# dgaddy/silent_speech

Measured on AMD Instinct MI355X. Metric: EMG frames/s training (transduction_model.py), higher is better.
Workload: dtype bf16

## Files before the change

### silent_speech_amd/csrc/loss.hip

```cpp
#include "common.h"
#include <stdlib.h>
#include "silent_speech_hip.h"
#include <math.h>

namespace {
constexpr int DESC = 10;
enum { D_N = 0, D_M, D_PRED_ROW0, D_TGT_ROW0, D_UNUSED, D_SK_OFF, D_DIRS_OFF, D_BND_OFF, D_RES_OFF };
constexpr int DW = 4, DR = 4;
__device__ __forceinline__ long long dtw_strips_d(long long n) { long long rows = n - 1, cap = DW * 64 * DR; return rows <= 0 ? 0 : (rows + cap - 1) / cap; }
__device__ __forceinline__ long long dtw_tsteps_d(long long m) { return m <= 1 ? 0 : (m - 1) + 63; }
}

__global__ void frame_lse_kernel(const float* __restrict__ head, long long ld, int col0, int ncls, int rows, float* __restrict__ lse, int* __restrict__ amax)
{
    const int lane = threadIdx.x & 63, wpb = blockDim.x >> 6;
    for (int r = blockIdx.x * wpb + (threadIdx.x >> 6); r < rows; r += gridDim.x * wpb) {
        const float* a = head + (long long)r * ld + col0;
        float mx = -INFINITY; int mi = 0x7fffffff;
        for (int c = lane; c < ncls; c += 64) { float v = a[c]; if (v > mx) { mx = v; mi = c; } }
        const float gmx = wave_max(mx);
        int cand = (mx == gmx) ? mi : 0x7fffffff;
#pragma unroll
        for (int m = 32; m >= 1; m >>= 1) { int o = __shfl_xor(cand, m); cand = o < cand ? o : cand; }
        float s = 0.f;
        for (int c = lane; c < ncls; c += 64) s += expf(a[c] - gmx);
        s = wave_sum(s);
        if (lane == 0) { lse[r] = gmx + logf(s); amax[r] = cand; }
    }
}

extern "C" int ss_frame_lse(const float* head, int64_t ld, int col0, int ncls, int rows, float* lse, int32_t* argmax, void* stream)
{
    SS_CHECK(head && lse && argmax, "ss_frame_lse: null pointer");
    if (rows <= 0) return 0;
    int blocks = (rows + 3) / 4; if (blocks > 4096) blocks = 4096;
    SS_LAUNCH(frame_lse_kernel, dim3(blocks), dim3(256), 0, stream, head, (long long)ld, col0, ncls, rows, lse, argmax);
    SS_LAUNCH_CHECK("ss_frame_lse");
    return 0;
}

constexpr int UTT = 8;
__global__ void loss_index_tables_kernel(const long long* __restrict__ utt, int* __restrict__ vo_pred, int* __restrict__ vo_tgt,
                                         int* __restrict__ si_tgt, int* __restrict__ si_base, int* __restrict__ si_res)
{
    const long long* u = utt + (long long)blockIdx.x * UTT;
    const int n1 = (int)u[0], n2 = (int)u[1];
    const int p0 = (int)u[3], t0 = (int)u[4], r0 = (int)u[5];
    if (u[2]) {
        const long long o = u[7];
        for (int i = threadIdx.x; i < n2; i += blockDim.x) { si_tgt[o + i] = t0 + i; si_base[o + i] = p0; si_res[o + i] = r0 + i; }
    } else {
        const long long o = u[6];
        for (int i = threadIdx.x; i < n1; i += blockDim.x) { vo_pred[o + i] = p0 + i; vo_tgt[o + i] = t0 + i; }
    }
}

extern "C" int ss_loss_index_tables(const int64_t* utt_dev, int n_utt, int32_t* vo_pred, int32_t* vo_tgt, int32_t* si_tgt, int32_t* si_base,
                                    int32_t* si_res, void* stream)
{
    SS_CHECK(n_utt >= 0, "ss_loss_index_tables: negative utterance count");
    if (n_utt == 0) return 0;
    SS_CHECK(utt_dev && vo_pred && vo_tgt && si_tgt && si_base && si_res, "ss_loss_index_tables: null pointer");
    SS_LAUNCH(loss_index_tables_kernel, dim3((unsigned)n_utt), dim3(256), 0, stream, (const long long*)utt_dev, (int*)vo_pred, (int*)vo_tgt, (int*)si_tgt,
              (int*)si_base, (int*)si_res);
    SS_LAUNCH_CHECK("ss_loss_index_tables");
    return 0;
}

__device__ __forceinline__ void loss_block_commit(float lsum, int csum, float inv_total, float* loss_acc, int* correct_acc)
{
    __shared__ float ls[16];
    __shared__ int cs[16];
    const int lane = threadIdx.x & 63, w = threadIdx.x >> 6, wpb = blockDim.x >> 6;
    if (lane == 0) { ls[w] = lsum; cs[w] = csum; }
    __syncthreads();
    if (threadIdx.x == 0) {
        float a = 0.f; int c = 0;
        for (int i = 0; i < wpb; ++i) { a += ls[i]; c += cs[i]; }
        if (a != 0.f) atomicAdd(loss_acc, a * inv_total);
        if (c) atomicAdd(correct_acc, c);
    }
}

__global__ void voiced_loss_kernel(const float* __restrict__ head, long long ld, int n_mel, int n_ph, const float* __restrict__ lse, const int* __restrict__ amax,
                                   const float* __restrict__ Y, const long long* __restrict__ phones, const int* __restrict__ pred_row, const int* __restrict__ tgt_row,
                                   int nframes, float lam, float inv_total, float* __restrict__ dhead, float* __restrict__ loss_acc, int* __restrict__ correct_acc)
{
    const int lane = threadIdx.x & 63, wpb = blockDim.x >> 6;
    float lsum = 0.f; int csum = 0;
    for (int f = blockIdx.x * wpb + (threadIdx.x >> 6); f < nframes; f += gridDim.x * wpb) {
        const int pr = pred_row[f], tr = tgt_row[f];
        const float* p = head + (long long)pr * ld; const float* y = Y + (long long)tr * n_mel;
        float* dp = dhead + (long long)pr * ld;
        float ss = 0.f;
        for (int c = lane; c < n_mel; c += 64) { float d = y[c] - p[c] + 1e-6f; ss += d * d; }
        const float dist = sqrtf(wave_sum(ss));
        const float gs = dist > 0.f ? inv_total / dist : 0.f;
        for (int c = lane; c < n_mel; c += 64) dp[c] = -(y[c] - p[c] + 1e-6f) * gs;
        const int ph = (int)phones[tr];
        const float L = lse[pr];
        for (int c = lane; c < n_ph; c += 64) dp[n_mel + c] = lam * inv_total * (expf(p[n_mel + c] - L) - (c == ph ? 1.f : 0.f));
        if (lane == 0) { lsum += dist + lam * (L - p[n_mel + ph]); csum += amax[pr] == ph; }
    }
    loss_block_commit(lsum, csum, inv_total, loss_acc, correct_acc);
}

extern "C" int ss_voiced_loss(const float* head, int64_t ld, int n_mel, int n_phone, const float* lse, const int32_t* argmax, const float* Y, const int64_t* phones,
                              const int32_t* pred_row, const int32_t* tgt_row, int nframes, float lam, float inv_total,
                              float* dhead, float* loss_accum, int32_t* correct_accum, void* stream)
{
    SS_CHECK(nframes >= 0, "ss_voiced_loss: negative frame count");
    if (nframes == 0) return 0;
    SS_CHECK(head && lse && argmax && Y && phones && pred_row && tgt_row && dhead && loss_accum && correct_accum, "ss_voiced_loss: null pointer");
    int blocks = (nframes + 3) / 4; if (blocks > 1024) blocks = 1024;
    SS_LAUNCH(voiced_loss_kernel, dim3(blocks), dim3(256), 0, stream, head, (long long)ld, n_mel, n_phone, lse, (const int*)argmax, Y, (const long long*)phones,
              (const int*)pred_row, (const int*)tgt_row, nframes, lam, inv_total, dhead, loss_accum, (int*)correct_accum);
    SS_LAUNCH_CHECK("ss_voiced_loss");
    return 0;
}

constexpr int YMAX = 128;
__device__ __forceinline__ float quad_bcast(float v, int k) {
#if defined(SS_EMU)
    return __shfl(v, (int)((threadIdx.x & 63) & ~3) + k);
#else
    switch (k) {
    case 0: return __int_as_float(__builtin_amdgcn_update_dpp(0, __float_as_int(v), 0x00, 0xf, 0xf, true));
    case 1: return __int_as_float(__builtin_amdgcn_update_dpp(0, __float_as_int(v), 0x55, 0xf, 0xf, true));
    case 2: return __int_as_float(__builtin_amdgcn_update_dpp(0, __float_as_int(v), 0xAA, 0xf, 0xf, true));
    default: return __int_as_float(__builtin_amdgcn_update_dpp(0, __float_as_int(v), 0xFF, 0xf, 0xf, true));
    }
#endif
}
template <int NQ>
__device__ __forceinline__ float quad_shared_sqdist(const float* __restrict__ p, int r, const f32x4 (&yv)[YMAX / 4]) {
    f32x4 own[NQ];
#pragma unroll
    for (int q = 0; q < NQ; ++q) own[q] = *(const f32x4*)(p + (r * NQ + q) * 4);
    float ss = 0.f;
#pragma unroll
    for (int k = 0; k < 4; ++k) {
#pragma unroll
        for (int q = 0; q < NQ; ++q) {
            const f32x4 b = yv[k * NQ + q];
            const float a0 = quad_bcast(own[q][0], k), a1 = quad_bcast(own[q][1], k), a2 = quad_bcast(own[q][2], k), a3 = quad_bcast(own[q][3], k);
            const float d0 = a0 - b[0], d1 = a1 - b[1], d2 = a2 - b[2], d3 = a3 - b[3];
            ss += d0 * d0; ss += d1 * d1; ss += d2 * d2; ss += d3 * d3;
        }
    }
    return ss;
}

__global__ __launch_bounds__(256) void silent_cost_skewed_kernel(const float* __restrict__ head, long long ld, int n_mel, const float* __restrict__ lse, const float* __restrict__ Y,
                                                                 const long long* __restrict__ phones, const long long* __restrict__ desc, float lam, unsigned char* __restrict__ ws, int* __restrict__ results, int CT)
{
    const long long* d = desc + (long long)blockIdx.y * DESC;
    const int N = (int)d[D_N], M = (int)d[D_M];
    const long long p0 = d[D_PRED_ROW0], y0 = d[D_TGT_ROW0];
    int* res = results + d[D_RES_OFF];
    for (int i = blockIdx.x * blockDim.x + threadIdx.x; i < N; i += gridDim.x * blockDim.x) res[i] = 0;
    const long long ts = dtw_tsteps_d(M), nkw = dtw_strips_d(N) * DW;
    if (ts <= 0) return;
    const long long tchunks = (ts + CT - 1) / CT, nwork = nkw * tchunks;
    float* sk = (float*)(ws + d[D_SK_OFF]);
    const int l = threadIdx.x >> 2, r = threadIdx.x & 3;
    for (long long wk = blockIdx.x; wk < nwork; wk += gridDim.x) {
        const long long kw = wk / tchunks, t0 = (wk - kw * tchunks) * CT;
        const long long i = 1 + (kw * 64 + l) * DR + r;
        const bool iv = i < N;
        f32x4 yv[YMAX / 4];
        int ph = 0;
        if (iv) {
            const float* y = Y + (y0 + i) * n_mel;
#pragma unroll
            for (int q = 0; q < YMAX / 4; ++q) if (q * 4 < n_mel) yv[q] = *(const f32x4*)(y + q * 4);
            ph = (int)phones[y0 + i];
        }
        const long long tend = t0 + CT < ts ? t0 + CT : ts;
        if (n_mel == 80) {
            for (long long t = t0; t < tend; ++t) {
                const long long j = t + 1 - l;
                const bool jv = j >= 1 && j < M;
                const float* p = head + (p0 + (jv ? j : 1)) * ld;
                const float ss = quad_shared_sqdist<5>(p, r, yv);
                float c = INFINITY;
                if (jv && iv) c = sqrtf(ss) + lam * (lse[p0 + j] - p[n_mel + ph]);
                sk[((kw * ts + t) * 64 + l) * DR + r] = c;
            }
            continue;
        }
        for (long long t = t0; t < tend; ++t) {
            const long long j = t + 1 - l;
            float c = INFINITY;
            if (iv && j >= 1 && j < M) {
                const float* p = head + (p0 + j) * ld;
                float ss = 0.f;
#pragma unroll
                for (int q = 0; q < YMAX / 4; ++q) {
                    if (q * 4 < n_mel) {
                        const f32x4 a = *(const f32x4*)(p + q * 4), b = yv[q];
                        const float d0 = a[0] - b[0], d1 = a[1] - b[1], d2 = a[2] - b[2], d3 = a[3] - b[3];
                        ss += d0 * d0; ss += d1 * d1; ss += d2 * d2; ss += d3 * d3;
                    }
                }
                c = sqrtf(ss) + lam * (lse[p0 + j] - p[n_mel + ph]);
            }
            sk[((kw * ts + t) * 64 + l) * DR + r] = c;
        }
    }
}

extern "C" int ss_silent_cost_skewed(const float* head, int64_t ld, int n_mel, const float* lse, const float* Y, const int64_t* phones,
                                     const int64_t* desc_dev, int n, int max_n, int max_m, float lam, void* workspace, int32_t* results, void* stream)
{
    SS_CHECK(n >= 0, "ss_silent_cost_skewed: negative batch");
    if (n == 0) return 0;
    SS_CHECK(head && lse && Y && phones && desc_dev && workspace && results, "ss_silent_cost_skewed: null pointer");
    SS_CHECK(n_mel % 4 == 0 && ld % 4 == 0, "ss_silent_cost_skewed: n_mel and ld must be multiples of 4 (16-byte rows)");
    SS_CHECK(n_mel <= YMAX, "ss_silent_cost_skewed: at most %d mel bins", YMAX);
    long long strips = max_n <= 1 ? 0 : (max_n - 1 + DW * 64 * DR - 1) / (DW * 64 * DR);
    const long long ts_max = max_m <= 1 ? 0 : max_m - 1 + 63;
    static const int CT = getenv("SS_COST_CT") ? atoi(getenv("SS_COST_CT")) : 16;
    long long blocks = strips * DW * ((ts_max + CT - 1) / CT);
    if (blocks < (max_n + 255) / 256) blocks = (max_n + 255) / 256;
    if (blocks > 4096) blocks = 4096;
    if (blocks < 1) blocks = 1;
    SS_LAUNCH(silent_cost_skewed_kernel, dim3((unsigned)blocks, n), dim3(256), 0, stream, head, (long long)ld, n_mel, lse, Y, (const long long*)phones,
              (const long long*)desc_dev, lam, (unsigned char*)workspace, (int*)results, CT);
    SS_LAUNCH_CHECK("ss_silent_cost_skewed");
    return 0;
}

__global__ void silent_loss_kernel(const float* __restrict__ head, long long ld, int n_mel, int n_ph, const float* __restrict__ lse, const int* __restrict__ amax,
                                   const float* __restrict__ Y, const long long* __restrict__ phones, const int* __restrict__ results,
                                   const int* __restrict__ tgt_row, const int* __restrict__ pred_base, const int* __restrict__ res_idx,
                                   int nframes, float lam, float inv_total, float* __restrict__ dhead, float* __restrict__ loss_acc, int* __restrict__ correct_acc)
{
    const int lane = threadIdx.x & 63, wpb = blockDim.x >> 6;
    float lsum = 0.f; int csum = 0;
    for (int f = blockIdx.x * wpb + (threadIdx.x >> 6); f < nframes; f += gridDim.x * wpb) {
        const int tr = tgt_row[f], pr = pred_base[f] + results[res_idx[f]];
        const float* p = head + (long long)pr * ld; const float* y = Y + (long long)tr * n_mel;
        float* dp = dhead + (long long)pr * ld;
        float ss = 0.f;
        for (int c = lane; c < n_mel; c += 64) { float d = p[c] - y[c]; ss += d * d; }
        const float dist = sqrtf(wave_sum(ss));
        const float gs = dist > 0.f ? inv_total / dist : 0.f;
        for (int c = lane; c < n_mel; c += 64) atomicAdd(dp + c, (p[c] - y[c]) * gs);
        const int ph = (int)phones[tr];
        const float L = lse[pr];
        for (int c = lane; c < n_ph; c += 64) atomicAdd(dp + n_mel + c, lam * inv_total * (expf(p[n_mel + c] - L) - (c == ph ? 1.f : 0.f)));
        if (lane == 0) { lsum += dist + lam * (L - p[n_mel + ph]); csum += amax[pr] == ph; }
    }
    loss_block_commit(lsum, csum, inv_total, loss_acc, correct_acc);
}

extern "C" int ss_silent_loss(const float* head, int64_t ld, int n_mel, int n_phone, const float* lse, const int32_t* argmax, const float* Y, const int64_t* phones,
                              const int32_t* results, const int32_t* tgt_row, const int32_t* pred_base, const int32_t* res_idx, int nframes,
                              float lam, float inv_total, float* dhead, float* loss_accum, int32_t* correct_accum, void* stream)
{
    SS_CHECK(nframes >= 0, "ss_silent_loss: negative frame count");
    if (nframes == 0) return 0;
    SS_CHECK(head && lse && argmax && Y && phones && results && tgt_row && pred_base && res_idx && dhead && loss_accum && correct_accum, "ss_silent_loss: null pointer");
    int blocks = (nframes + 3) / 4; if (blocks > 1024) blocks = 1024;
    SS_LAUNCH(silent_loss_kernel, dim3(blocks), dim3(256), 0, stream, head, (long long)ld, n_mel, n_phone, lse, (const int*)argmax, Y, (const long long*)phones,
              (const int*)results, (const int*)tgt_row, (const int*)pred_base, (const int*)res_idx, nframes, lam, inv_total, dhead, loss_accum, (int*)correct_accum);
    SS_LAUNCH_CHECK("ss_silent_loss");
    return 0;
}

__global__ void phoneme_confusion_kernel(const int* __restrict__ amax, const long long* __restrict__ phones, const int* __restrict__ results,
                                         const int* __restrict__ vo_pred, const int* __restrict__ vo_tgt, int n_voiced,
                                         const int* __restrict__ si_tgt, const int* __restrict__ si_base, const int* __restrict__ si_res, int n_silent,
                                         int* __restrict__ conf, int n_phone)
{
    for (int i = blockIdx.x * blockDim.x + threadIdx.x; i < n_voiced + n_silent; i += gridDim.x * blockDim.x) {
        int p, t;
        if (i < n_voiced) { p = amax[vo_pred[i]]; t = (int)phones[vo_tgt[i]]; }
        else { const int k = i - n_voiced; p = amax[si_base[k] + results[si_res[k]]]; t = (int)phones[si_tgt[k]]; }
        if ((unsigned)p < (unsigned)n_phone && (unsigned)t < (unsigned)n_phone) atomicAdd(conf + p * n_phone + t, 1);
        else atomicAdd(conf + n_phone * n_phone, 1);
    }
}

extern "C" int ss_phoneme_confusion(const int32_t* argmax, const int64_t* phones, const int32_t* results, const int32_t* vo_pred, const int32_t* vo_tgt,
                                    int n_voiced, const int32_t* si_tgt, const int32_t* si_base, const int32_t* si_res, int n_silent_frames,
                                    int32_t* confusion, int n_phone, void* stream)
{
    SS_CHECK(argmax && phones && confusion, "ss_phoneme_confusion: null pointer");
    SS_CHECK(n_voiced == 0 || (vo_pred && vo_tgt), "ss_phoneme_confusion: voiced tables missing");
    SS_CHECK(n_silent_frames == 0 || (results && si_tgt && si_base && si_res), "ss_phoneme_confusion: silent tables missing");
    const int n = n_voiced + n_silent_frames;
    if (n <= 0) return 0;
    int blocks = (n + 255) / 256; if (blocks > 1024) blocks = 1024;
    SS_LAUNCH(phoneme_confusion_kernel, dim3(blocks), dim3(256), 0, stream, argmax, (const long long*)phones, results, vo_pred, vo_tgt, n_voiced,
              si_tgt, si_base, si_res, n_silent_frames, confusion, n_phone);
    SS_LAUNCH_CHECK("ss_phoneme_confusion");
    return 0;
}
```

### silent_speech_amd/csrc/runtime.hip

```cpp
#include "common.h"
#include "silent_speech_hip.h"
#include <stdarg.h>

static thread_local char g_err[512] = "";

void ss_set_error(const char* fmt, ...) {
    va_list ap; va_start(ap, fmt);
    vsnprintf(g_err, sizeof(g_err), fmt, ap);
    va_end(ap);
}
extern "C" const char* ss_last_error(void) { return g_err; }
extern "C" int ss_abi_version(void) { return SS_ABI_VERSION; }
extern "C" const char* ss_target_arch(void) {
#if defined(SS_EMU)
    return "host-emulator";
#else
    return "gfx950";
#endif
}
int ss_check_launch(const char* what) {
    hipError_t e = hipGetLastError();
    if (e != hipSuccess) { ss_set_error("%s: kernel launch failed: %s", what, hipGetErrorString(e)); return 2; }
    return 0;
}

#if !defined(SS_EMU)
#include <mutex>
namespace {
struct PinnedRing {
    static constexpr int N = 8;
    void* buf[N] = {}; size_t cap[N] = {}; hipEvent_t ev[N] = {}; bool used[N] = {}; int at = 0; std::mutex mu;
};
PinnedRing g_ring;
}
#endif
int ss_upload_table(void* dst_dev, const void* src_host, size_t bytes, void* stream)
{
    if (bytes == 0) return 0;
#if defined(SS_EMU)
    memcpy(dst_dev, src_host, bytes);
    return 0;
#else
    std::lock_guard<std::mutex> lock(g_ring.mu);
    const int i = g_ring.at; g_ring.at = (i + 1) % PinnedRing::N;
    if (g_ring.used[i] && hipEventSynchronize(g_ring.ev[i]) != hipSuccess) { ss_set_error("table upload: event wait failed"); return 1; }
    if (g_ring.cap[i] < bytes) {
        if (g_ring.buf[i]) (void)hipHostFree(g_ring.buf[i]);
        size_t cap = 1 << 16; while (cap < bytes) cap <<= 1;
        if (hipHostMalloc(&g_ring.buf[i], cap, hipHostMallocDefault) != hipSuccess) { g_ring.buf[i] = nullptr; g_ring.cap[i] = 0; ss_set_error("table upload: pinned allocation of %zu bytes failed", cap); return 1; }
        g_ring.cap[i] = cap;
    }
    if (!g_ring.ev[i] && hipEventCreateWithFlags(&g_ring.ev[i], hipEventDisableTiming) != hipSuccess) { ss_set_error("table upload: event creation failed"); return 1; }
    memcpy(g_ring.buf[i], src_host, bytes);
    if (hipMemcpyAsync(dst_dev, g_ring.buf[i], bytes, hipMemcpyHostToDevice, (hipStream_t)stream) != hipSuccess) { ss_set_error("table upload failed"); return 1; }
    if (hipEventRecord(g_ring.ev[i], (hipStream_t)stream) != hipSuccess) { ss_set_error("table upload: event record failed"); return 1; }
    g_ring.used[i] = true;
    return 0;
#endif
}

template <class TI, class TO>
__global__ void permute3d_kernel(const TI* __restrict__ in, TO* __restrict__ out, int d0, int d1, int d2,
                                 long long s0, long long s1, long long s2, int valid1, int valid2, float scale, int accumulate)
{
    long long total = (long long)d0 * d1 * d2;
    for (long long i = (long long)blockIdx.x * blockDim.x + threadIdx.x; i < total; i += (long long)gridDim.x * blockDim.x) {
        int c = (int)(i % d2); long long t = i / d2; int b = (int)(t % d1); int a = (int)(t / d1);
        float v = (b < valid1 && c < valid2) ? ldf(in + a * s0 + b * s1 + c * s2) * scale : 0.f;
        if (accumulate) v += ldf(out + i);
        stf(out + i, v);
    }
}

extern "C" int ss_permute3d(const void* in, int in_dtype, void* out, int out_dtype, int d0, int d1, int d2,
                            int64_t s0, int64_t s1, int64_t s2, int valid1, int valid2, float scale, int accumulate, void* stream)
{
    SS_CHECK(in && out, "ss_permute3d: null pointer");
    SS_CHECK(d0 >= 0 && d1 >= 0 && d2 >= 0, "ss_permute3d: negative extent");
    long long total = (long long)d0 * d1 * d2;
    if (total == 0) return 0;
    int block = 256; long long g = (total + block - 1) / block; if (g > 4096) g = 4096;
    dim3 grid((unsigned)g), blk(block);
#define SS_P3(TI, TO) SS_LAUNCH(SS_KERNEL(permute3d_kernel<TI, TO>), grid, blk, 0, stream, (const TI*)in, (TO*)out, d0, d1, d2, (long long)s0, (long long)s1, (long long)s2, valid1, valid2, scale, accumulate)
    if (in_dtype == SS_F32 && out_dtype == SS_F32) SS_P3(float, float);
    else if (in_dtype == SS_F32 && out_dtype == SS_BF16) SS_P3(float, bf16_t);
    else if (in_dtype == SS_BF16 && out_dtype == SS_F32) SS_P3(bf16_t, float);
    else if (in_dtype == SS_BF16 && out_dtype == SS_BF16) SS_P3(bf16_t, bf16_t);
    else SS_CHECK(false, "ss_permute3d: bad dtype");
#undef SS_P3
    SS_LAUNCH_CHECK("ss_permute3d");
    return 0;
}

struct PermuteJob {
    const void* in; void* out;
    long long s0, s1, s2, o0, o1;
    int d0, d1, d2, valid1, valid2, in_dtype, out_dtype, accumulate;
    float scale; int first_block, nblocks, pad_;
};

template <class TI> struct Vec4;
template <> struct Vec4<float> { static __device__ __forceinline__ void load(const float* p, float (&v)[4]) { const f32x4 a = *(const f32x4*)p; v[0] = a[0]; v[1] = a[1]; v[2] = a[2]; v[3] = a[3]; } };
template <> struct Vec4<bf16_t> { static __device__ __forceinline__ void load(const bf16_t* p, float (&v)[4]) { const u32x2 a = *(const u32x2*)p; v[0] = __uint_as_float(a[0] << 16); v[1] = __uint_as_float(a[0] & 0xffff0000u); v[2] = __uint_as_float(a[1] << 16); v[3] = __uint_as_float(a[1] & 0xffff0000u); } };

template <class TI, class TO, bool GROUPED_RMW = false>
__device__ __forceinline__ void permute_job(const PermuteJob& j, int lb, int nthreads, int tid, float* tile)
{
    const long long total = (long long)j.d0 * j.d1 * j.d2;
    const TI* in = (const TI*)j.in; TO* out = (TO*)j.out;
    const long long as0 = j.s0 < 0 ? -j.s0 : j.s0, as1 = j.s1 < 0 ? -j.s1 : j.s1, as2 = j.s2 < 0 ? -j.s2 : j.s2;
    const bool c0 = j.d0 > 1 && as0 >= 1 && as0 <= 4, c1 = j.d1 > 1 && as1 >= 1 && as1 <= 4;
    const bool fx1 = c1 && (!c0 || j.d1 >= j.d0), fx0 = c0 && !fx1;
    const int dXq = fx1 ? j.d1 : j.d0;
    const bool al16 = ((uintptr_t)in % 16) == 0 && ((uintptr_t)out % 16) == 0;
    if (!GROUPED_RMW && !j.accumulate && j.s2 == 1 && j.s1 == j.d2 && j.o1 == j.d2 && (j.d0 == 1 || (j.s0 == (long long)j.d1 * j.d2 && j.o0 == j.s0)) &&
        j.valid1 >= j.d1 && j.valid2 >= j.d2 && (total & 7) == 0 && al16 && total < (1LL << 34)) {
        const unsigned n8 = (unsigned)(total >> 3), step = (unsigned)j.nblocks * nthreads;
        for (unsigned i = (unsigned)lb * nthreads + tid; i < n8; i += step) {
            float v[8]; Vec8<TI>::load(in + (size_t)i * 8, v);
#pragma unroll
            for (int e = 0; e < 8; ++e) v[e] *= j.scale;
            Vec8<TO>::store(out + (size_t)i * 8, v);
        }
        return;
    }
    if (!GROUPED_RMW && sizeof(TO) == 2 && !j.accumulate && as2 >= 8 && (fx0 || fx1) && nthreads == 256 && al16) {
        const int dX = fx1 ? j.d1 : j.d0, dO = fx1 ? j.d0 : j.d1;
        const long long sX = fx1 ? j.s1 : j.s0, sO = fx1 ? j.s0 : j.s1, oX = fx1 ? j.o1 : j.o0, oO = fx1 ? j.o0 : j.o1;
        const int vX = fx1 ? (j.valid1 < j.d1 ? j.valid1 : j.d1) : dX, vO = fx1 ? dO : (j.valid1 < j.d1 ? j.valid1 : j.d1), vC = j.valid2 < j.d2 ? j.valid2 : j.d2;
        if (sX == 1 && !(dX & 7) && !(j.d2 & 7) && !(sO & 7) && !(j.s2 & 7) && !(oX & 7) && !(oO & 7) && !(vX & 7) && !(vC & 7) && dX >= 64 && j.d2 >= 64) {
            unsigned short* t16 = (unsigned short*)tile;
            const int tiles_x = (dX + 63) >> 6, tiles_c = (j.d2 + 63) >> 6;
            const long long ntiles = (long long)dO * tiles_x * tiles_c;
            for (long long t = lb; t < ntiles; t += j.nblocks) {
                const int oi = (int)(t / (tiles_x * tiles_c)), rem = (int)(t - (long long)oi * (tiles_x * tiles_c));
                const int tx = rem / tiles_c, tc = rem - tx * tiles_c;
#pragma unroll
                for (int k = 0; k < 2; ++k) {
                    const int f = k * 256 + tid, cc = f >> 3, x0 = (f & 7) * 8, gx = tx * 64 + x0, gc = tc * 64 + cc;
                    float v[8] = {0.f, 0.f, 0.f, 0.f, 0.f, 0.f, 0.f, 0.f};
                    if (gx < vX && gc < vC && oi < vO) { Vec8<TI>::load(in + oi * sO + gx + (long long)gc * j.s2, v);
#pragma unroll
                        for (int e = 0; e < 8; ++e) v[e] *= j.scale; }
                    unsigned* d = (unsigned*)(t16 + cc * 66 + x0);
#pragma unroll
                    for (int e = 0; e < 4; ++e) d[e] = pack_bf16(v[2 * e], v[2 * e + 1]);
                }
                __syncthreads();
#pragma unroll
                for (int k = 0; k < 2; ++k) {
                    const int f = k * 256 + tid, x = f >> 3, c0 = (f & 7) * 8, gx = tx * 64 + x, gc = tc * 64 + c0;
                    if (gx < dX && gc < j.d2) {
                        u32x4 r;
#pragma unroll
                        for (int e = 0; e < 4; ++e) r[e] = (unsigned)t16[(c0 + 2 * e) * 66 + x] | ((unsigned)t16[(c0 + 2 * e + 1) * 66 + x] << 16);
                        *(u32x4*)(out + oi * oO + gx * oX + gc) = r;
                    }
                }
                __syncthreads();
            }
            return;
        }
    }
    if (sizeof(TI) == 4 && sizeof(TO) == 4 && as2 >= 4 && (fx0 || fx1) && nthreads == 256 && al16) {
        const int dX = fx1 ? j.d1 : j.d0, dO = fx1 ? j.d0 : j.d1;
        const long long sX = fx1 ? j.s1 : j.s0, sO = fx1 ? j.s0 : j.s1, oX = fx1 ? j.o1 : j.o0, oO = fx1 ? j.o0 : j.o1;
        const int vX = fx1 ? (j.valid1 < j.d1 ? j.valid1 : j.d1) : dX, vO = fx1 ? dO : (j.valid1 < j.d1 ? j.valid1 : j.d1), vC = j.valid2 < j.d2 ? j.valid2 : j.d2;
        if (sX == 1 && !(dX & 3) && !(j.d2 & 3) && !(sO & 3) && !(j.s2 & 3) && !(oX & 3) && !(oO & 3) && !(vX & 3) && !(vC & 3) && dX >= 32 && j.d2 >= 32) {
            const int tiles_x = (dX + 63) >> 6, tiles_c = (j.d2 + 63) >> 6;
            const long long ntiles = (long long)dO * tiles_x * tiles_c;
            for (long long t = lb; t < ntiles; t += j.nblocks) {
                const int oi = (int)(t / (tiles_x * tiles_c)), rem = (int)(t - (long long)oi * (tiles_x * tiles_c));
                const int tx = rem / tiles_c, tc = rem - tx * tiles_c;
                f32x4 v[4];
#pragma unroll
                for (int k = 0; k < 4; ++k) {
                    const int f = k * 256 + tid, cc = f >> 4, x0 = (f & 15) * 4, gx = tx * 64 + x0, gc = tc * 64 + cc;
                    const f32x4 z = {0.f, 0.f, 0.f, 0.f};
                    v[k] = (gx < vX && gc < vC && oi < vO) ? *(const f32x4*)((const float*)in + oi * sO + gx + (long long)gc * j.s2) : z;
                }
#pragma unroll
                for (int k = 0; k < 4; ++k) {
                    const int f = k * 256 + tid, cc = f >> 4, x0 = (f & 15) * 4;
#pragma unroll
                    for (int e = 0; e < 4; ++e) tile[cc * 65 + x0 + e] = v[k][e] * j.scale;
                }
                __syncthreads();
                f32x4 w[4]; float* op[4];
#pragma unroll
                for (int k = 0; k < 4; ++k) {
                    const int f = k * 256 + tid, x = f >> 4, c0 = (f & 15) * 4, gx = tx * 64 + x, gc = tc * 64 + c0;
                    op[k] = (gx < dX && gc < j.d2) ? (float*)out + oi * oO + gx * oX + gc : nullptr;
                    const f32x4 z = {0.f, 0.f, 0.f, 0.f};
                    w[k] = (op[k] && j.accumulate) ? *(const f32x4*)op[k] : z;
                }
#pragma unroll
                for (int k = 0; k < 4; ++k) {
                    const int f = k * 256 + tid, x = f >> 4, c0 = (f & 15) * 4;
                    if (op[k]) {
#pragma unroll
                        for (int e = 0; e < 4; ++e) w[k][e] += tile[(c0 + e) * 65 + x];
                        *(f32x4*)op[k] = w[k];
                    }
                }
                __syncthreads();
            }
            return;
        }
    }
    if (as2 > 4 && (fx0 || fx1) && nthreads == 256 && total >= 4096 && (long long)(dXq < 64 ? dXq : 64) * (j.d2 < 64 ? j.d2 : 64) >= 192) {
        const int dX = fx1 ? j.d1 : j.d0, dO = fx1 ? j.d0 : j.d1;
        const long long sX = fx1 ? j.s1 : j.s0, sO = fx1 ? j.s0 : j.s1, oX = fx1 ? j.o1 : j.o0, oO = fx1 ? j.o0 : j.o1;
        const int lx = dX <= 4 ? 2 : (dX <= 16 ? 4 : (j.d2 <= 4 ? 10 : (j.d2 <= 16 ? 8 : 6)));
        const int TX = 1 << lx, lc = 12 - lx, TC = 1 << lc, P = TX + 1;
        const int tiles_x = (dX + TX - 1) >> lx, tiles_c = (j.d2 + TC - 1) >> lc;
        const long long ntiles = (long long)dO * tiles_x * tiles_c;
        for (long long t = lb; t < ntiles; t += j.nblocks) {
            const int oi = (int)(t / (tiles_x * tiles_c)), rem = (int)(t - (long long)oi * (tiles_x * tiles_c));
            const int tx = rem / tiles_c, tc = rem - tx * tiles_c;
            {
                float v[16];
#pragma unroll
                for (int k = 0; k < 16; ++k) {
                    const int f = k * 256 + tid, x = f & (TX - 1), cc = f >> lx;
                    const int gx = tx * TX + x, gc = tc * TC + cc, bb = fx1 ? gx : oi;
                    v[k] = 0.f;
                    if (gx < dX && gc < j.d2 && bb < j.valid1 && gc < j.valid2) v[k] = ldf(in + oi * sO + gx * sX + (long long)gc * j.s2) * j.scale;
                }
#pragma unroll
                for (int k = 0; k < 16; ++k) { const int f = k * 256 + tid; tile[(f >> lx) * P + (f & (TX - 1))] = v[k]; }
            }
            __syncthreads();
            if (!GROUPED_RMW || !j.accumulate) {
#pragma unroll
                for (int k = 0; k < 16; ++k) {
                    const int f = k * 256 + tid, x = f >> lc, cc = f & (TC - 1);
                    const int gx = tx * TX + x, gc = tc * TC + cc;
                    if (gx < dX && gc < j.d2) {
                        TO* o = out + oi * oO + gx * oX + gc;
                        float w = tile[cc * P + x];
                        if (j.accumulate) w += ldf(o);
                        stf(o, w);
                    }
                }
            } else {
#pragma unroll
                for (int h = 0; h < 2; ++h) {
                    float w[8];
#pragma unroll
                    for (int k = 0; k < 8; ++k) {
                        const int f = (h * 8 + k) * 256 + tid, x = f >> lc, cc = f & (TC - 1);
                        const int gx = tx * TX + x, gc = tc * TC + cc;
                        w[k] = tile[cc * P + x];
                        if (gx < dX && gc < j.d2) w[k] += ldf(out + oi * oO + gx * oX + gc);
                    }
#pragma unroll
                    for (int k = 0; k < 8; ++k) {
                        const int f = (h * 8 + k) * 256 + tid, x = f >> lc, cc = f & (TC - 1);
                        const int gx = tx * TX + x, gc = tc * TC + cc;
                        if (gx < dX && gc < j.d2) stf(out + oi * oO + gx * oX + gc, w[k]);
                    }
                }
            }
            __syncthreads();
        }
        return;
    }
    if (j.s2 == 1 && !(j.d2 & 3) && !(j.s0 & 3) && !(j.s1 & 3) && !(j.o0 & 3) && !(j.o1 & 3) && !(j.valid2 & 3) &&
        ((uintptr_t)in % (4 * sizeof(TI))) == 0 && ((uintptr_t)out % (4 * sizeof(TO))) == 0) {
        const int c4n = j.d2 >> 2;
        for (long long i = (long long)lb * nthreads + tid; i < (total >> 2); i += (long long)j.nblocks * nthreads) {
            const int c = (int)(i % c4n) * 4; const long long t = i / c4n; const int b = (int)(t % j.d1); const int a = (int)(t / j.d1);
            float v[4] = {0.f, 0.f, 0.f, 0.f};
            if (b < j.valid1 && c < j.valid2) { Vec4<TI>::load(in + a * j.s0 + b * j.s1 + c, v); v[0] *= j.scale; v[1] *= j.scale; v[2] *= j.scale; v[3] *= j.scale; }
            TO* o = out + a * j.o0 + b * j.o1 + c;
            if (j.accumulate) { float w[4]; Vec4<TO>::load(o, w); v[0] += w[0]; v[1] += w[1]; v[2] += w[2]; v[3] += w[3]; }
            if (sizeof(TO) == 4) { const f32x4 r = {v[0], v[1], v[2], v[3]}; *(f32x4*)o = r; }
            else { const u32x2 r = {pack_bf16(v[0], v[1]), pack_bf16(v[2], v[3])}; *(u32x2*)o = r; }
        }
        return;
    }
    for (long long i = (long long)lb * nthreads + tid; i < total; i += (long long)j.nblocks * nthreads) {
        const int c = (int)(i % j.d2); const long long t = i / j.d2; const int b = (int)(t % j.d1); const int a = (int)(t / j.d1);
        float v = (b < j.valid1 && c < j.valid2) ? ldf(in + a * j.s0 + b * j.s1 + c * j.s2) * j.scale : 0.f;
        TO* o = out + a * j.o0 + b * j.o1 + c;
        if (j.accumulate) v += ldf(o);
        stf(o, v);
    }
}

__global__ void permute3d_batch_kernel(const PermuteJob* __restrict__ jobs, const int* __restrict__ job_of_block)
{
    __shared__ float tile[1024 * 5];
    const PermuteJob j = jobs[job_of_block[blockIdx.x]];
    const int lb = blockIdx.x - j.first_block;
    if (j.in_dtype == SS_F32 && j.out_dtype == SS_F32) permute_job<float, float>(j, lb, blockDim.x, threadIdx.x, tile);
    else if (j.in_dtype == SS_F32) permute_job<float, bf16_t>(j, lb, blockDim.x, threadIdx.x, tile);
    else if (j.out_dtype == SS_F32) permute_job<bf16_t, float>(j, lb, blockDim.x, threadIdx.x, tile);
    else permute_job<bf16_t, bf16_t>(j, lb, blockDim.x, threadIdx.x, tile);
}

__global__ __launch_bounds__(256) void permute3d_batch_f32_kernel(const PermuteJob* __restrict__ jobs, const int* __restrict__ job_of_block)
{
    __shared__ float tile[1024 * 5];
    const PermuteJob j = jobs[job_of_block[blockIdx.x]];
    permute_job<float, float, true>(j, blockIdx.x - j.first_block, blockDim.x, threadIdx.x, tile);
}

extern "C" int ss_permute3d_batch(const void* jobs_dev, const int32_t* job_of_block_dev, int total_blocks, int all_f32, void* stream)
{
    SS_CHECK(total_blocks >= 0, "ss_permute3d_batch: negative block count");
    if (total_blocks == 0) return 0;
    SS_CHECK(jobs_dev && job_of_block_dev, "ss_permute3d_batch: null pointer");
    if (all_f32) SS_LAUNCH(permute3d_batch_f32_kernel, dim3(total_blocks), dim3(256), 0, stream, (const PermuteJob*)jobs_dev, (const int*)job_of_block_dev);
    else SS_LAUNCH(permute3d_batch_kernel, dim3(total_blocks), dim3(256), 0, stream, (const PermuteJob*)jobs_dev, (const int*)job_of_block_dev);
    SS_LAUNCH_CHECK("ss_permute3d_batch");
    return 0;
}
```

Before: 1.698 million.

## Specialize DTW cost kernel by mel width and add LDS-staged small-permute path

```diff
diff --git a/silent_speech_amd/csrc/loss.hip b/silent_speech_amd/csrc/loss.hip
--- a/silent_speech_amd/csrc/loss.hip
+++ b/silent_speech_amd/csrc/loss.hip
@@ -132,25 +132,33 @@
     }
 #endif
 }
-template <int NQ>
-__device__ __forceinline__ float quad_shared_sqdist(const float* __restrict__ p, int r, const f32x4 (&yv)[YMAX / 4]) {
-    f32x4 own[NQ];
-#pragma unroll
-    for (int q = 0; q < NQ; ++q) own[q] = *(const f32x4*)(p + (r * NQ + q) * 4);
-    float ss = 0.f;
+template <int NQ, int U>
+__device__ __forceinline__ void quad_shared_sqdist(const float* const (&p)[U], int r, const f32x4 (&yv)[4 * NQ], float (&ss)[U]) {
+    f32x4 own[U][NQ];
+#pragma unroll
+    for (int u = 0; u < U; ++u) {
+#pragma unroll
+        for (int q = 0; q < NQ; ++q) own[u][q] = *(const f32x4*)(p[u] + (r * NQ + q) * 4);
+    }
+#pragma unroll
+    for (int u = 0; u < U; ++u) ss[u] = 0.f;
 #pragma unroll
     for (int k = 0; k < 4; ++k) {
 #pragma unroll
         for (int q = 0; q < NQ; ++q) {
             const f32x4 b = yv[k * NQ + q];
-            const float a0 = quad_bcast(own[q][0], k), a1 = quad_bcast(own[q][1], k), a2 = quad_bcast(own[q][2], k), a3 = quad_bcast(own[q][3], k);
-            const float d0 = a0 - b[0], d1 = a1 - b[1], d2 = a2 - b[2], d3 = a3 - b[3];
-            ss += d0 * d0; ss += d1 * d1; ss += d2 * d2; ss += d3 * d3;
+#pragma unroll
+            for (int u = 0; u < U; ++u) {
+                const float a0 = quad_bcast(own[u][q][0], k), a1 = quad_bcast(own[u][q][1], k), a2 = quad_bcast(own[u][q][2], k), a3 = quad_bcast(own[u][q][3], k);
+                const float d0 = a0 - b[0], d1 = a1 - b[1], d2 = a2 - b[2], d3 = a3 - b[3];
+                ss[u] = fmaf(d0, d0, ss[u]); ss[u] = fmaf(d1, d1, ss[u]); ss[u] = fmaf(d2, d2, ss[u]); ss[u] = fmaf(d3, d3, ss[u]);
+            }
         }
     }
-    return ss;
-}
-
+}
+constexpr int CU = 1;
+
+template <int NY>
 __global__ __launch_bounds__(256) void silent_cost_skewed_kernel(const float* __restrict__ head, long long ld, int n_mel, const float* __restrict__ lse, const float* __restrict__ Y,
                                                                  const long long* __restrict__ phones, const long long* __restrict__ desc, float lam, unsigned char* __restrict__ ws, int* __restrict__ results, int CT)
 {
@@ -168,44 +176,53 @@
         const long long kw = wk / tchunks, t0 = (wk - kw * tchunks) * CT;
         const long long i = 1 + (kw * 64 + l) * DR + r;
         const bool iv = i < N;
-        f32x4 yv[YMAX / 4];
+        f32x4 yv[NY];
         int ph = 0;
         if (iv) {
             const float* y = Y + (y0 + i) * n_mel;
 #pragma unroll
-            for (int q = 0; q < YMAX / 4; ++q) if (q * 4 < n_mel) yv[q] = *(const f32x4*)(y + q * 4);
+            for (int q = 0; q < NY; ++q) if (q * 4 < n_mel) yv[q] = *(const f32x4*)(y + q * 4);
             ph = (int)phones[y0 + i];
         }
         const long long tend = t0 + CT < ts ? t0 + CT : ts;
-        if (n_mel == 80) {
+        if constexpr (NY == 20) {
+            for (long long t = t0; t < tend; t += CU) {
+                const float* p[CU]; bool jv[CU]; float ph_term[CU], ss[CU];
+#pragma unroll
+                for (int u = 0; u < CU; ++u) {
+                    const long long j = t + u + 1 - l;
+                    jv[u] = t + u < tend && j >= 1 && j < M;
+                    p[u] = head + (p0 + (jv[u] ? j : 1)) * ld;
+                    ph_term[u] = (jv[u] && iv) ? lse[p0 + j] - p[u][n_mel + ph] : 0.f;
+                }
+                quad_shared_sqdist<5, CU>(p, r, yv, ss);
+#pragma unroll
+                for (int u = 0; u < CU; ++u) {
+                    if (t + u >= tend) break;
+                    float c = INFINITY;
+                    if (jv[u] && iv) c = sqrtf(ss[u]) + lam * ph_term[u];
+                    sk[((kw * ts + t + u) * 64 + l) * DR + r] = c;
+                }
+            }
+        } else {
             for (long long t = t0; t < tend; ++t) {
                 const long long j = t + 1 - l;
-                const bool jv = j >= 1 && j < M;
-                const float* p = head + (p0 + (jv ? j : 1)) * ld;
-                const float ss = quad_shared_sqdist<5>(p, r, yv);
                 float c = INFINITY;
-                if (jv && iv) c = sqrtf(ss) + lam * (lse[p0 + j] - p[n_mel + ph]);
+                if (iv && j >= 1 && j < M) {
+                    const float* p = head + (p0 + j) * ld;
+                    float ss = 0.f;
+#pragma unroll
+                    for (int q = 0; q < NY; ++q) {
+                        if (q * 4 < n_mel) {
+                            const f32x4 a = *(const f32x4*)(p + q * 4), b = yv[q];
+                            const float d0 = a[0] - b[0], d1 = a[1] - b[1], d2 = a[2] - b[2], d3 = a[3] - b[3];
+                            ss += d0 * d0; ss += d1 * d1; ss += d2 * d2; ss += d3 * d3;
+                        }
+                    }
+                    c = sqrtf(ss) + lam * (lse[p0 + j] - p[n_mel + ph]);
+                }
                 sk[((kw * ts + t) * 64 + l) * DR + r] = c;
             }
-            continue;
-        }
-        for (long long t = t0; t < tend; ++t) {
-            const long long j = t + 1 - l;
-            float c = INFINITY;
-            if (iv && j >= 1 && j < M) {
-                const float* p = head + (p0 + j) * ld;
-                float ss = 0.f;
-#pragma unroll
-                for (int q = 0; q < YMAX / 4; ++q) {
-                    if (q * 4 < n_mel) {
-                        const f32x4 a = *(const f32x4*)(p + q * 4), b = yv[q];
-                        const float d0 = a[0] - b[0], d1 = a[1] - b[1], d2 = a[2] - b[2], d3 = a[3] - b[3];
-                        ss += d0 * d0; ss += d1 * d1; ss += d2 * d2; ss += d3 * d3;
-                    }
-                }
-                c = sqrtf(ss) + lam * (lse[p0 + j] - p[n_mel + ph]);
-            }
-            sk[((kw * ts + t) * 64 + l) * DR + r] = c;
         }
     }
 }
@@ -225,8 +242,10 @@
     if (blocks < (max_n + 255) / 256) blocks = (max_n + 255) / 256;
     if (blocks > 4096) blocks = 4096;
     if (blocks < 1) blocks = 1;
-    SS_LAUNCH(silent_cost_skewed_kernel, dim3((unsigned)blocks, n), dim3(256), 0, stream, head, (long long)ld, n_mel, lse, Y, (const long long*)phones,
-              (const long long*)desc_dev, lam, (unsigned char*)workspace, (int*)results, CT);
+    if (n_mel == 80) SS_LAUNCH(silent_cost_skewed_kernel<20>, dim3((unsigned)blocks, n), dim3(256), 0, stream, head, (long long)ld, n_mel, lse, Y, (const long long*)phones,
+                               (const long long*)desc_dev, lam, (unsigned char*)workspace, (int*)results, CT);
+    else SS_LAUNCH(silent_cost_skewed_kernel<YMAX / 4>, dim3((unsigned)blocks, n), dim3(256), 0, stream, head, (long long)ld, n_mel, lse, Y, (const long long*)phones,
+                   (const long long*)desc_dev, lam, (unsigned char*)workspace, (int*)results, CT);
     SS_LAUNCH_CHECK("ss_silent_cost_skewed");
     return 0;
 }
diff --git a/silent_speech_amd/csrc/runtime.hip b/silent_speech_amd/csrc/runtime.hip
--- a/silent_speech_amd/csrc/runtime.hip
+++ b/silent_speech_amd/csrc/runtime.hip
@@ -103,6 +103,10 @@
 template <> struct Vec4<float> { static __device__ __forceinline__ void load(const float* p, float (&v)[4]) { const f32x4 a = *(const f32x4*)p; v[0] = a[0]; v[1] = a[1]; v[2] = a[2]; v[3] = a[3]; } };
 template <> struct Vec4<bf16_t> { static __device__ __forceinline__ void load(const bf16_t* p, float (&v)[4]) { const u32x2 a = *(const u32x2*)p; v[0] = __uint_as_float(a[0] << 16); v[1] = __uint_as_float(a[0] & 0xffff0000u); v[2] = __uint_as_float(a[1] << 16); v[3] = __uint_as_float(a[1] & 0xffff0000u); } };
 
+template <class TO> __device__ __forceinline__ void ldo(const TO* p, float (&v)[16 / sizeof(TO)]) {
+    if constexpr (sizeof(TO) == 4) Vec4<TO>::load(p, v); else Vec8<TO>::load(p, v);
+}
+
 template <class TI, class TO, bool GROUPED_RMW = false>
 __device__ __forceinline__ void permute_job(const PermuteJob& j, int lb, int nthreads, int tid, float* tile)
 {
@@ -124,6 +128,51 @@
         }
         return;
     }
+    {
+        constexpr int VO = 16 / (int)sizeof(TO), CAP = 1024 * 5, NV = (CAP / VO + 255) / 256;
+        const long long R = (long long)j.d1 * j.d2;
+        if (nthreads == 256 && j.d1 > 1 && j.d2 > 1 && j.s1 == 1 && j.s2 == j.d1 && j.o1 == j.d2 && (j.d0 == 1 || (j.s0 == R && j.o0 == R)) &&
+            j.valid1 >= j.d1 && j.valid2 >= j.d2 && R <= CAP && !(R & 7) && al16) {
+            const int Ri = (int)R, G = CAP / Ri, nch = (j.d0 + G - 1) / G;
+            for (int ch = lb; ch < nch; ch += j.nblocks) {
+                const int a0 = ch * G, n = (j.d0 - a0 < G ? j.d0 - a0 : G) * Ri;
+                const TI* src = in + (long long)a0 * R; TO* dst = out + (long long)a0 * R;
+                for (int i = tid * 4; i < n; i += 1024) {
+                    float v[4]; Vec4<TI>::load(src + i, v);
+                    const f32x4 r = {v[0] * j.scale, v[1] * j.scale, v[2] * j.scale, v[3] * j.scale};
+                    *(f32x4*)(tile + i) = r;
+                }
+                __syncthreads();
+                float acc[GROUPED_RMW ? NV : 1][VO];
+                if (GROUPED_RMW && j.accumulate) {
+#pragma unroll
+                    for (int k = 0; k < NV; ++k) {
+                        const int p = (k * 256 + tid) * VO;
+                        if (p < n) ldo(dst + p, acc[GROUPED_RMW ? k : 0]);
+                    }
+                }
+#pragma unroll
+                for (int k = 0; k < NV; ++k) {
+                    const int p = (k * 256 + tid) * VO;
+                    if (p < n) {
+                        int s = p / Ri; const int pr = p - s * Ri; int b = pr / j.d2, c = pr - b * j.d2;
+                        float w[VO];
+                        if (!GROUPED_RMW && j.accumulate) ldo(dst + p, acc[0]);
+#pragma unroll
+                        for (int e = 0; e < VO; ++e) {
+                            w[e] = tile[s * Ri + c * j.d1 + b];
+                            if (j.accumulate) w[e] += acc[GROUPED_RMW ? k : 0][e];
+                            if (++c == j.d2) { c = 0; if (++b == j.d1) { b = 0; ++s; } }
+                        }
+                        if constexpr (sizeof(TO) == 4) { const f32x4 r = {w[0], w[1], w[2], w[3]}; *(f32x4*)(dst + p) = r; }
+                        else Vec8<TO>::store(dst + p, w);
+                    }
+                }
+                __syncthreads();
+            }
+            return;
+        }
+    }
     if (!GROUPED_RMW && sizeof(TO) == 2 && !j.accumulate && as2 >= 8 && (fx0 || fx1) && nthreads == 256 && al16) {
         const int dX = fx1 ? j.d1 : j.d0, dO = fx1 ? j.d0 : j.d1;
         const long long sX = fx1 ? j.s1 : j.s0, sO = fx1 ? j.s0 : j.s1, oX = fx1 ? j.o1 : j.o0, oO = fx1 ? j.o0 : j.o1;
```

New measurement: 1.707 million, median of 6. No clear change (+0.5%).
